# apasarkar/localmd

Hardware: AMD Instinct MI355X
Metric: frames/sec PMD decomposition (higher is better)
Workload: dtype f32; 1 GPU; 512x512x10000_b20; frames=10000, block=20, frames_to_init=10000, max_components=50, parallelism=1 process per GPU

## Files before the change

include/pmd_hip.h:

```cpp
#ifndef PMD_HIP_H
#define PMD_HIP_H
#include <stddef.h>
#include <stdint.h>

#ifdef __cplusplus
extern "C" {
#endif

typedef struct pmd_ctx pmd_ctx;

int pmd_version(void);
int pmd_ctx_create(int device, void* hip_stream, pmd_ctx** out);
int pmd_ctx_destroy(pmd_ctx* ctx);
int pmd_ctx_set_stream(pmd_ctx* ctx, void* hip_stream);
int pmd_ctx_sync(pmd_ctx* ctx);
const char* pmd_last_error(pmd_ctx* ctx);

int pmd_profile_enable(pmd_ctx* ctx, int on);
int pmd_profile_query(pmd_ctx* ctx, const char* name, double* total_ms, int* count);
int pmd_profile_names(pmd_ctx* ctx, char* buf, int cap);

int pmd_tile_dpad(int d);
int pmd_tile_rpad(int r);
long pmd_time_ld(long t);
// ... 101 lines not shown
                      float* R_out, long ldr, float* s_out, float* Vt_out, long ldvt, void* ws, size_t ws_bytes);
int pmd_gram_blocks(pmd_ctx* ctx, const float* Uw, int dpad, int b1, int b2, const int* tile_pix, const int* pairs,
                    int n_pairs, const int* origins, const int* col_off, const int* ranks, int n_tiles, int Rt,
                    const float* basis, long D, int K, float* Gblk, float* Gbg, float* Gstrip, long ldgs);
int pmd_gram_apply(pmd_ctx* ctx, const float* Gblk, const float* Gbg, const float* Gstrip, long ldgs, const int* nbr_ptr,
                   const int* nbr, const int* col_off, const int* ranks, int n_tiles, int Rt, int K, int max_rank,
                   const float* M, long ldm, int ncols, float* GM, long ldgm);
size_t pmd_orthogonalize_factored_workspace_bytes(int m);
int pmd_orthogonalize_factored(pmd_ctx* ctx, const float* M, int Rc, int m, long ldm, const float* GM, long ldgm,
                               float* Et_out, long lde, int* rprime_host, void* ws, size_t ws_bytes);
int pmd_orthogonalize_chol(pmd_ctx* ctx, const float* M, int Rc, int m, long ldm, const float* GM, long ldgm,
                           float* Et_out, long lde, int* ok_host, void* ws, size_t ws_bytes);
size_t pmd_orthogonalize_chol_workspace_bytes(int Rc, int m);
int pmd_psvd_vp_gram(pmd_ctx* ctx, const float* Et, int rp, int m, long lde, const float* W1, int nc, long ldw, int et_lower, float* Vp,
                     long ldv, float* C, long ldc);
size_t pmd_psvd_finish_workspace_bytes(int rp);
int pmd_psvd_finish(pmd_ctx* ctx, float* C, long ldc, int rp, const float* Vp, int nc, long ldv, float* W_out, long ldw, float* s_out,
                    float* Vt_out, long ldvt, void* ws, size_t ws_bytes);
size_t pmd_projected_svd_factored_workspace_bytes(int Rc, int m, int rp, int T);
int pmd_projected_svd_factored(pmd_ctx* ctx, const float* M, int Rc, int m, long ldm, const float* Et, int rp, long lde,
                               const float* Z, int T, long ldz, float* R_out, long ldr, float* s_out, float* Vt_out,
                               long ldvt, float* Vp_out, long ldvp, float* X1_out, const float* W1_in, int et_lower,
                               void* ws, size_t ws_bytes);
size_t pmd_gram_mtgm_workspace_bytes(int rows, int m);
long pmd_gram_mtgm_ld(int rows);
int pmd_gram_mtgm(pmd_ctx* ctx, const float* M, int rows, int m, long ldm, const float* GM, long ldgm, float* C, long ldc,
                  void* ws, size_t ws_bytes);
size_t pmd_chol_inverse_workspace_bytes(int m);
int pmd_chol_inverse(pmd_ctx* ctx, float* C, int m, long ldc, int abs_last_pivot, int* ok_host, void* ws, size_t ws_bytes);
int pmd_transpose(pmd_ctx* ctx, const float* src, long ld_src, int rows, int cols, float* dst, long ld_dst);
// ... 60 lines not shown
```

localmd_amd/_lib.py:

```python
import ctypes as C
import os

_HERE = os.path.dirname(os.path.abspath(__file__))
LIB_PATH = os.environ.get("PMD_HIP_LIB") or os.path.join(_HERE, "libpmd_hip.so")

c_i, c_l, c_f, c_d, c_p = C.c_int, C.c_long, C.c_float, C.c_double, C.c_void_p
c_u64, c_u32, c_sz = C.c_uint64, C.c_uint32, C.c_size_t

SIGNATURES = {
    "pmd_version": (c_i, []),
    "pmd_comm_unique_id": (c_i, [c_p]),
    "pmd_ctx_create": (c_i, [c_i, c_p, C.POINTER(c_p)]),
    "pmd_ctx_destroy": (c_i, [c_p]),
    "pmd_ctx_set_stream": (c_i, [c_p, c_p]),
    "pmd_ctx_sync": (c_i, [c_p]),
    "pmd_last_error": (C.c_char_p, [c_p]),
    "pmd_profile_enable": (c_i, [c_p, c_i]),
    "pmd_profile_query": (c_i, [c_p, C.c_char_p, C.POINTER(c_d), C.POINTER(c_i)]),
    "pmd_profile_names": (c_i, [c_p, C.c_char_p, c_i]),
    "pmd_tile_dpad": (c_i, [c_i]),
    "pmd_tile_rpad": (c_i, [c_i]),
    "pmd_time_ld": (c_l, [c_l]),
    "pmd_rng_normal": (c_i, [c_p, c_u64, c_u32, c_u32, c_u32, c_i, c_l, c_i, c_i, c_p, c_l, c_l]),
    "pmd_stats_workspace_bytes": (c_sz, [c_i, c_l, c_i]),
# ... 56 lines not shown
    "pmd_projected_svd_factored_workspace_bytes": (c_sz, [c_i, c_i, c_i, c_i]),
    "pmd_projected_svd_factored": (c_i, [c_p, c_p, c_i, c_i, c_l, c_p, c_i, c_l, c_p, c_i, c_l, c_p, c_l, c_p, c_p, c_l,
                                         c_p, c_l, c_p, c_p, c_i, c_p, c_sz]),
    "pmd_gram_mtgm_workspace_bytes": (c_sz, [c_i, c_i]),
    "pmd_gram_mtgm_ld": (c_l, [c_i]),
    "pmd_gram_mtgm": (c_i, [c_p, c_p, c_i, c_i, c_l, c_p, c_l, c_p, c_l, c_p, c_sz]),
    "pmd_chol_inverse_workspace_bytes": (c_sz, [c_i]),
    "pmd_chol_inverse": (c_i, [c_p, c_p, c_i, c_l, c_i, C.POINTER(c_i), c_p, c_sz]),
    "pmd_ctx_set_null_cutoff": (c_i, [c_p, C.c_float]),
    "pmd_comm_init": (c_i, [c_p, c_p, c_i, c_i]),
    "pmd_comm_destroy": (c_i, [c_p]),
    "pmd_comm_all_reduce_f32": (c_i, [c_p, c_p, c_sz]),
    "pmd_comm_all_gather": (c_i, [c_p, c_p, c_p, c_sz]),
    "pmd_transpose": (c_i, [c_p, c_p, c_l, c_i, c_i, c_p, c_l]),
    "pmd_psvd_vp_gram": (c_i, [c_p, c_p, c_i, c_i, c_l, c_p, c_i, c_l, c_i, c_p, c_l, c_p, c_l]),
    "pmd_psvd_finish_workspace_bytes": (c_sz, [c_i]),
    "pmd_psvd_finish": (c_i, [c_p, c_p, c_l, c_i, c_p, c_i, c_l, c_p, c_l, c_p, c_p, c_l, c_p, c_sz]),
    "pmd_csr_count": (c_i, [c_p, c_i, c_i, c_i, c_p, c_p, c_i, c_p, c_i, c_p]),
    "pmd_csr_fill": (c_i, [c_p, c_i, c_i, c_i, c_i, c_p, c_p, c_p, c_p, c_i, c_p, c_p, c_p, c_i, c_p, c_p, c_p, c_i, c_i,
                           c_p, c_p, c_p, c_p, c_i]),
    "pmd_scratch_trim": (c_i, [c_p, C.c_size_t]),
    "pmd_gemm_split_active": (c_i, [c_p, c_i, c_i, c_i]),
    "pmd_gemm": (c_i, [c_p, c_i, c_i, c_i, c_i, c_i, c_f, c_p, c_l, c_p, c_l, c_f, c_p, c_l]),
    "pmdk_tile_atx": (c_i, [c_p, c_p, c_l, c_p, c_i, c_l, c_i, c_p, c_l, c_i, c_p, c_l, c_l, c_i, c_i, c_i]),
    "pmdk_tile_atx_rows": (c_i, [c_p, c_p, c_l, c_p, c_i, c_l, c_i, c_p, c_l, c_i, c_p, c_l, c_l, c_i, c_i, c_i, c_i]),
    "pmdk_tile_xbt": (c_i, [c_p, c_p, c_l, c_p, c_i, c_l, c_i, c_p, c_l, c_l, c_p, c_l, c_l, c_i, c_i, c_i, c_i]),
    "pmdk_tile_gram": (c_i, [c_p, c_p, c_l, c_l, c_i, c_i, c_i, c_p]),
    "pmdk_tile_rowmix": (c_i, [c_p, c_p, c_l, c_l, c_p, c_l, c_i, c_i, c_p, c_l, c_l, c_i, c_i]),
    "pmdk_small_qr": (c_i, [c_p, c_p, c_l, c_i, c_i, c_i, c_p, c_l, c_i, c_i]),
    "pmdk_small_eig": (c_i, [c_p, c_p, c_i, c_i, c_i, c_d, c_p, c_p, c_i]),
# ... 138 lines not shown
```

localmd_amd/csrc/capi.hip:

```cpp
#include "pmd_internal.h"
#include "../../include/pmd_hip.h"

#define CTX_CHECK(ctx) \
  if (!(ctx)) return PMD_ERR_ARG;

extern "C" {

int pmd_version(void) { return 1; }

int pmd_ctx_create(int device, void* hip_stream, pmd_ctx** out) {
  if (!out) return PMD_ERR_ARG;
  *out = nullptr;
  int count = 0;
  if (hipGetDeviceCount(&count) != hipSuccess || device < 0 || device >= count) return PMD_ERR_HIP;
  if (hipSetDevice(device) != hipSuccess) return PMD_ERR_HIP;
  pmd_ctx* ctx = new pmd_ctx();
  ctx->device = device;
  ctx->stream = (hipStream_t)hip_stream;
  ctx->tables = nullptr;
  ctx->scratch = nullptr;
  ctx->scratch_bytes = 0;
  ctx->scratch2 = nullptr;
  ctx->scratch2_bytes = 0;
  ctx->atx_ranks = nullptr;
// ... 406 lines not shown
size_t pmd_chol_inverse_workspace_bytes(int m) { return pmd_chol_inverse_workspace_bytes_impl(m); }
int pmd_chol_inverse(pmd_ctx* ctx, float* C, int m, long ldc, int abs_last_pivot, int* ok_host, void* ws, size_t ws_bytes) {
  CTX_CHECK(ctx);
  return pmd_chol_inverse_impl(ctx, C, m, ldc, abs_last_pivot, ok_host, ws, ws_bytes);
}
int pmd_transpose(pmd_ctx* ctx, const float* src, long ld_src, int rows, int cols, float* dst, long ld_dst) {
  CTX_CHECK(ctx);
  return pmd_transpose_impl(ctx, src, ld_src, rows, cols, dst, ld_dst);
}
int pmd_psvd_vp_gram(pmd_ctx* ctx, const float* Et, int rp, int m, long lde, const float* W1, int nc, long ldw, int et_lower, float* Vp,
                     long ldv, float* C, long ldc) {
  CTX_CHECK(ctx);
  if (rp < 1 || m < rp || nc < 0 || ldc < rp) return pmd_fail(ctx, PMD_ERR_ARG, "pmd_psvd_vp_gram", "bad shape");
  return pmd_psvd_vp_gram_impl(ctx, Et, rp, m, lde, W1, nc, ldw, et_lower, Vp, ldv, C, ldc);
}
size_t pmd_psvd_finish_workspace_bytes(int rp) { return pmd_psvd_finish_workspace_bytes_impl(rp); }
int pmd_psvd_finish(pmd_ctx* ctx, float* C, long ldc, int rp, const float* Vp, int nc, long ldv, float* W_out, long ldw, float* s_out,
                    float* Vt_out, long ldvt, void* ws, size_t ws_bytes) {
  CTX_CHECK(ctx);
  if (rp < 1 || nc < 0 || ldc < rp) return pmd_fail(ctx, PMD_ERR_ARG, "pmd_psvd_finish", "bad shape");
  return pmd_psvd_finish_impl(ctx, C, ldc, rp, Vp, nc, ldv, W_out, ldw, s_out, Vt_out, ldvt, ws, ws_bytes);
}
size_t pmd_projected_svd_factored_workspace_bytes(int Rc, int m, int rp, int T) {
  return pmd_projected_svd_factored_workspace_bytes_impl(Rc, m, rp, T);
}
int pmd_projected_svd_factored(pmd_ctx* ctx, const float* M, int Rc, int m, long ldm, const float* Et, int rp, long lde,
                               const float* Z, int T, long ldz, float* R_out, long ldr, float* s_out, float* Vt_out,
                               long ldvt, float* Vp_out, long ldvp, float* X1_out, const float* W1_in, int et_lower,
                               void* ws, size_t ws_bytes) {
  CTX_CHECK(ctx);
// ... 96 lines not shown
```

localmd_amd/csrc/global.hip:

```cpp
#include "pmd_internal.h"
#include <rocsolver/rocsolver.h>
#include <algorithm>
#include <cmath>
#include <vector>

#define RUN(call)                 \
  do {                            \
    int rc__ = (call);            \
    if (rc__ != PMD_OK) return rc__; \
  } while (0)

#define PMD_BLAS(ctx, call)                                                     \
  do {                                                                          \
    rocblas_status s__ = (call);                                                \
    if (s__ != rocblas_status_success) return pmd_fail(ctx, PMD_ERR_BLAS, #call, rocblas_status_to_string(s__)); \
  } while (0)

__global__ void sum_partials_kernel(const float* __restrict__ part, long mn, int n, int S, float beta, float* __restrict__ C, long ldc) {
  for (long i = blockIdx.x * (long)blockDim.x + threadIdx.x; i < mn; i += (long)gridDim.x * blockDim.x) {
    const long r = i / n;
    const int c = (int)(i - r * n);
    float acc = 0.f;
    for (int s = 0; s < S; ++s) acc += part[(long)s * mn + i];
    float* o = C + r * ldc + c;
// ... 356 lines not shown
  PMD_HIP(ctx, hipMemcpyAsync(scale, hscale.data(), (size_t)rp * sizeof(float), hipMemcpyHostToDevice, ctx->stream));
  RUN(launch_gather_rows(ctx, C, ldc, perm, scale, rp, m, Et, m));
  if (M) RUN(pmd_gemm_rm(ctx, 0, 1, R, rp, m, 1.f, M, ldm, Et, m, 0.f, P_out, ldp));
  else RUN(launch_transpose(ctx, Et, m, rp, m, P_out, ldp));
  PMD_HIP(ctx, hipStreamSynchronize(ctx->stream));
  return PMD_OK;
}

size_t pmd_projected_svd_workspace_bytes_impl(int rows_p, int n1, int n2) {
  const size_t nk = (size_t)std::min(n1, n2);
  size_t b = (nk + 4) * nk * sizeof(float) * 2 + nk * (sizeof(float) * 5 + sizeof(int)) + 8192;
  if (n1 > n2) b += (size_t)n1 * n2 * sizeof(float);
  return b + 8192;
}

int pmd_projected_svd_impl(pmd_ctx* ctx, const float* P, int rows_p, long ldp, const float* V, int n1, int n2, long ldv,
                           float* R_out, long ldr, float* s_out, float* Vt_out, long ldvt, void* ws, size_t ws_bytes) {
  const int nk = std::min(n1, n2);
  pmd_arena ar(ws, ws_bytes);
  const long ldc = pmd_round_up(nk, 4);
  float* C = ar.take_n<float>((size_t)ldc * nk);
  float* Wt = ar.take_n<float>((size_t)nk * nk);
  float* w = ar.take_n<float>(nk);
  float* work = ar.take_n<float>(nk);
  float* sgn = ar.take_n<float>(nk);
  float* inv = ar.take_n<float>(nk);
  int* perm = ar.take_n<int>(nk);
  int* info = ar.take_n<int>(4);
  float* left = (n1 > n2) ? ar.take_n<float>((size_t)n1 * n2) : nullptr;
  if (ar.overflow) return pmd_fail(ctx, PMD_ERR_WORKSPACE, "pmd_projected_svd", "workspace too small");
  {
    pmd_prof_scope prof__(ctx, "rocblas_ssyrk");
    const float one = 1.f, zero = 0.f;
    const int kfull = (n1 <= n2) ? n2 : n1;
    const int kc = pmd_gemm_k_chunk(kfull);
    for (int k0 = 0; k0 < kfull; k0 += kc) {
      const int kk = std::min(kc, kfull - k0);
      if (n1 <= n2)
        PMD_BLAS(ctx, rocblas_ssyrk(ctx->blas, rocblas_fill_lower, rocblas_operation_transpose, n1, kk, &one, V + k0, (rocblas_int)ldv,
                                    k0 == 0 ? &zero : &one, C, (rocblas_int)ldc));
      else
        PMD_BLAS(ctx, rocblas_ssyrk(ctx->blas, rocblas_fill_lower, rocblas_operation_none, n2, kk, &one, V + (long)k0 * ldv, (rocblas_int)ldv,
                                    k0 == 0 ? &zero : &one, C, (rocblas_int)ldc));
    }
  }
  RUN(pmd_syevd(ctx, nk, C, ldc, w, work, info));
  std::vector<float> hw(nk);
  int hinfo = 0;
  PMD_HIP(ctx, hipMemcpyAsync(hw.data(), w, (size_t)nk * sizeof(float), hipMemcpyDeviceToHost, ctx->stream));
  PMD_HIP(ctx, hipMemcpyAsync(&hinfo, info, sizeof(int), hipMemcpyDeviceToHost, ctx->stream));
  PMD_HIP(ctx, hipStreamSynchronize(ctx->stream));
  if (hinfo != 0) return pmd_fail(ctx, PMD_ERR_BLAS, "rocsolver_ssyevd", "did not converge");
  std::vector<int> idx(nk);
  for (int i = 0; i < nk; ++i) idx[i] = i;
  std::stable_sort(idx.begin(), idx.end(), [&](int a, int b) { return std::fabs(hw[a]) > std::fabs(hw[b]); });
  std::vector<float> hs(nk), hsgn(nk), hinv(nk);
  for (int i = 0; i < nk; ++i) {
    const float lam = hw[idx[i]];
// ... 11 lines not shown
    hipLaunchKernelGGL(scale_rows2_kernel, dim3(8, nk), dim3(256), 0, ctx->stream, Vt_out, ldvt, n2, inv);
    PMD_LAUNCH_CHECK(ctx, "scale_rows2_kernel");
    if (P) RUN(pmd_gemm_rm(ctx, 0, 1, rows_p, nk, n1, 1.f, P, ldp, Wt, nk, 0.f, R_out, ldr));
    else RUN(launch_transpose(ctx, Wt, nk, nk, n1, R_out, ldr));
  } else {
    RUN(pmd_gemm_rm(ctx, 0, 1, n1, nk, n2, 1.f, V, ldv, Wt, nk, 0.f, left, nk));
    hipLaunchKernelGGL(scale_cols_kernel, dim3(8, n1), dim3(256), 0, ctx->stream, left, (long)nk, nk, inv);
    PMD_LAUNCH_CHECK(ctx, "scale_cols_kernel");
    RUN(pmd_gemm_rm(ctx, 0, 0, rows_p, nk, n1, 1.f, P, ldp, left, nk, 0.f, R_out, ldr));
    PMD_HIP(ctx, hipMemcpy2DAsync(Vt_out, ldvt * sizeof(float), Wt, (size_t)nk * sizeof(float), (size_t)nk * sizeof(float), nk, hipMemcpyDeviceToDevice, ctx->stream));
  }
  PMD_HIP(ctx, hipStreamSynchronize(ctx->stream));
  return PMD_OK;
}

static int psvd_gram_rows(pmd_ctx* ctx, const float* V, int n1, int n2, long ldv, float* C, long ldc) {
  pmd_prof_scope prof__(ctx, "rocblas_ssyrk");
  const float one = 1.f, zero = 0.f;
  const int kc = pmd_gemm_k_chunk(n2);
  if (n2 <= 0) { PMD_HIP(ctx, hipMemsetAsync(C, 0, (size_t)n1 * ldc * sizeof(float), ctx->stream)); return PMD_OK; }
  for (int k0 = 0; k0 < n2; k0 += kc) {
    const int kk = std::min(kc, n2 - k0);
    PMD_BLAS(ctx, rocblas_ssyrk(ctx->blas, rocblas_fill_lower, rocblas_operation_transpose, n1, kk, &one, V + k0, (rocblas_int)ldv,
                                k0 == 0 ? &zero : &one, C, (rocblas_int)ldc));
  }
  return PMD_OK;
}

int pmd_psvd_vp_gram_impl(pmd_ctx* ctx, const float* Et, int rp, int m, long lde, const float* W1, int nc, long ldw, int et_lower,
                          float* Vp, long ldv, float* C, long ldc) {
  if (nc > 0) {
    const bool tri = et_lower && rp == m && !pmd_f16x2_wanted(ctx, rp, nc, m);
    const float one = 1.f;
    if (tri) {
      pmd_prof_scope prof__(ctx, "rocblas_strmm");
      PMD_BLAS(ctx, rocblas_strmm(ctx->blas, rocblas_side_right, rocblas_fill_upper, rocblas_operation_none, rocblas_diagonal_non_unit, nc, m,
                                  &one, Et, (rocblas_int)lde, W1, (rocblas_int)ldw, Vp, (rocblas_int)ldv));
    } else {
      RUN(pmd_gemm_rm(ctx, 0, 0, rp, nc, m, 1.f, Et, lde, W1, ldw, 0.f, Vp, ldv));
    }
  }
  return psvd_gram_rows(ctx, Vp, rp, nc, ldv, C, ldc);
}

size_t pmd_psvd_finish_workspace_bytes_impl(int rp) {
  return (size_t)rp * rp * sizeof(float) + (size_t)rp * (sizeof(float) * 5 + sizeof(int)) + 16384;
}

int pmd_psvd_finish_impl(pmd_ctx* ctx, float* C, long ldc, int rp, const float* Vp, int nc, long ldv, float* W_out, long ldw, float* s_out,
                         float* Vt_out, long ldvt, void* ws, size_t ws_bytes) {
  pmd_arena ar(ws, ws_bytes);
  float* Wt = ar.take_n<float>((size_t)rp * rp);
  float* w = ar.take_n<float>(rp);
  float* work = ar.take_n<float>(rp);
  float* sgn = ar.take_n<float>(rp);
  float* inv = ar.take_n<float>(rp);
  int* perm = ar.take_n<int>(rp);
// ... 503 lines not shown
  pmd_arena ar(ws, ws_bytes);
  float* W1 = ar.take_n<float>((size_t)m * T);
  float* Vp = Vp_out ? Vp_out : ar.take_n<float>((size_t)rp * T);
  const long ldv = Vp_out ? ldvp : T;
  float* X1 = X1_out ? X1_out : ar.take_n<float>((size_t)m * rp);
  const long ldt = pmd_round_up(Rc, 64);
  float* Mt = ar.take_n<float>((size_t)m * ldt);
  const size_t sub_bytes = pmd_projected_svd_workspace_bytes_impl(1, rp, T);
  void* sub = ar.take(sub_bytes);
  if (ar.overflow) return pmd_fail(ctx, PMD_ERR_WORKSPACE, "pmd_projected_svd_factored", "workspace too small");
  if (!W1_in) {
    RUN(launch_transpose(ctx, M, ldm, Rc, m, Mt, ldt));
    RUN(pmd_gemm_rm(ctx, 0, 0, m, T, Rc, 1.f, Mt, ldt, Z, ldz, 0.f, W1, T));
  }
  const bool tri_any = et_lower && rp == m;
  const bool tri = tri_any && !pmd_f16x2_wanted(ctx, rp, T, m);
  const float one = 1.f;
  if (tri) {
    pmd_prof_scope prof__(ctx, "rocblas_strmm");
    PMD_BLAS(ctx, rocblas_strmm(ctx->blas, rocblas_side_right, rocblas_fill_upper, rocblas_operation_none,
                                rocblas_diagonal_non_unit, T, m, &one, Et, (rocblas_int)lde, W1_in ? W1_in : W1, T, Vp,
                                (rocblas_int)ldv));
  } else {
    RUN(pmd_gemm_rm(ctx, 0, 0, rp, T, m, 1.f, Et, lde, W1_in ? W1_in : W1, T, 0.f, Vp, ldv));
  }
  float* Wmat = W1;
  RUN(pmd_projected_svd_impl(ctx, nullptr, 0, 0, Vp, rp, T, ldv, Wmat, rp, s_out, Vt_out, ldvt, sub, sub_bytes));
  if (tri_any && !pmd_f16x2_wanted(ctx, m, rp, rp)) {
    pmd_prof_scope prof__(ctx, "rocblas_strmm");
    PMD_BLAS(ctx, rocblas_strmm(ctx->blas, rocblas_side_right, rocblas_fill_upper, rocblas_operation_transpose,
                                rocblas_diagonal_non_unit, rp, m, &one, Et, (rocblas_int)lde, Wmat, rp, X1, rp));
  } else {
    RUN(pmd_gemm_rm(ctx, 1, 0, m, rp, rp, 1.f, Et, lde, Wmat, rp, 0.f, X1, rp));
  }
  if (R_out) RUN(pmd_gemm_rm(ctx, 0, 0, Rc, rp, m, 1.f, M, ldm, X1, rp, 0.f, R_out, ldr));
  return PMD_OK;
}

#define CHOL_NB 128
#define CHOL_LS (CHOL_NB + 1)
__global__ __launch_bounds__(256) void potf2_block_kernel(float* __restrict__ A, long ld, int nb, int k0, int* __restrict__ info,
                                                          int n_abs_last, float* __restrict__ linv_out) {
  extern __shared__ float chol_dyn[];
  __shared__ float s_col[2][CHOL_NB];
  const int tid = threadIdx.x;
  const int tr = tid >> 4, tc = tid & 15;
  float a[8][8];
#pragma unroll
  for (int i = 0; i < 8; ++i)
// ... 431 lines not shown
```

localmd_amd/csrc/pmd_internal.h:

```cpp
#pragma once
#include "pmd_common.h"

int pmd_init_tables(pmd_ctx* ctx);
extern "C" {
int pmd_tile_dpad(int d);
long pmd_time_ld(long t);
size_t pmd_stats_workspace_bytes(int T, long D, int frame_const);
size_t pmd_stats_stream_workspace_bytes(int T, long D);
}

int pmd_launch_rng(pmd_ctx* ctx, uint64_t seed, uint32_t stream, uint32_t index0, uint32_t index_step, int batch,
                   long rows, int cols, int transpose, float* out, long ld, long batch_stride);

int pmd_launch_stats(pmd_ctx* ctx, const float* movie, int T, long D, int frame_const, int do_noise, float* mean_out,
                     float* std_out, void* ws, size_t ws_bytes);
int pmd_launch_standardize_transpose(pmd_ctx* ctx, const float* movie, long D, const int* frames, int nf,
                                     const float* mean, const float* stdv, float* out, long ld);
int pmd_launch_stats_stream_accumulate(pmd_ctx* ctx, const void* batch, int elem, int t0, int nb, int T, long D,
                                       int do_noise, void* ws, size_t ws_bytes);
int pmd_launch_stats_stream_finish(pmd_ctx* ctx, int T, long D, int do_noise, float* mean_out, float* std_out, void* ws,
                                   size_t ws_bytes);
int pmd_launch_standardize_transpose_typed(pmd_ctx* ctx, const void* movie, int elem, long D, const int* frames, int nf,
                                           const float* mean, const float* stdv, float* out, long ld);
int pmd_launch_gather_frames(pmd_ctx* ctx, const void* src, int elem, long D, const int* src_rows, const int* dst_rows,
// ... 152 lines not shown
int pmd_csr_fill_impl(pmd_ctx* ctx, int d1, int d2, int order_f, int b1, const int* cover1, const int* cover2,
                      const int* orig1, const int* orig2, int n2, const int* ranks, const int* col_off, const float* Ut,
                      int dpad, const float* w, const double* inv_cumw, const float* basis, int K, int Rt,
                      const long* indptr, double* data, int* indices, int* zero_count, int rpad);
size_t pmd_orthogonalize_factored_workspace_bytes_impl(int m);
int pmd_orthogonalize_factored_impl(pmd_ctx* ctx, const float* M, int Rc, int m, long ldm, const float* GM, long ldgm,
                                    float* Et_out, long lde, int* rprime_out, void* ws, size_t ws_bytes);
size_t pmd_projected_svd_factored_workspace_bytes_impl(int Rc, int m, int rp, int T);
size_t pmd_orthogonalize_chol_workspace_bytes_impl(int Rc, int m);
int pmd_projected_svd_factored_impl(pmd_ctx* ctx, const float* M, int Rc, int m, long ldm, const float* Et, int rp,
                                    long lde, const float* Z, int T, long ldz, float* R_out, long ldr, float* s_out,
                                    float* Vt_out, long ldvt, float* Vp_out, long ldvp, float* X1_out,
                                    const float* W1_in, int et_lower, void* ws, size_t ws_bytes);
int pmd_psvd_vp_gram_impl(pmd_ctx* ctx, const float* Et, int rp, int m, long lde, const float* W1, int nc, long ldw, int et_lower,
                          float* Vp, long ldv, float* C, long ldc);
size_t pmd_psvd_finish_workspace_bytes_impl(int rp);
int pmd_psvd_finish_impl(pmd_ctx* ctx, float* C, long ldc, int rp, const float* Vp, int nc, long ldv, float* W_out, long ldw, float* s_out,
                         float* Vt_out, long ldvt, void* ws, size_t ws_bytes);
long pmd_gram_mtgm_ld_impl(int rows);
size_t pmd_gram_mtgm_workspace_bytes_impl(int rows, int m);
int pmd_gram_mtgm_impl(pmd_ctx* ctx, const float* M, int rows, int m, long ldm, const float* GM, long ldgm, float* C,
                       long ldc, void* ws, size_t ws_bytes);
size_t pmd_chol_inverse_workspace_bytes_impl(int m);
int pmd_chol_inverse_impl(pmd_ctx* ctx, float* C, int m, long ldc, int abs_last_pivot, int* ok_host, void* ws, size_t ws_bytes);
int pmd_transpose_impl(pmd_ctx* ctx, const float* src, long lds_, int rows, int cols, float* dst, long ldd);
int pmd_orthogonalize_chol_impl(pmd_ctx* ctx, const float* M, int Rc, int m, long ldm, const float* GM, long ldgm,
                                float* Et_out, long lde, int* ok_host, void* ws, size_t ws_bytes);

int pmd_launch_bin_average(pmd_ctx* ctx, const float* X, long ldx, long n_rows, int a, int nbins, float* xbar, long ldb);
int pmd_launch_tile_cross_gram(pmd_ctx* ctx, const float* A, const float* B, long tile_stride, int ld, int len,
// ... 15 lines not shown
```

localmd_amd/csrc/sytrd.hip:

```cpp
#include "pmd_internal.h"
#include <rocsolver/rocsolver.h>
#include <algorithm>
#include <cmath>
#include <cstdlib>
#include <vector>

#define PMD_BLAS(ctx, call)                                                     \
  do {                                                                          \
    rocblas_status s__ = (call);                                                \
    if (s__ != rocblas_status_success) return pmd_fail(ctx, PMD_ERR_BLAS, #call, rocblas_status_to_string(s__)); \
  } while (0)

namespace {

constexpr int NB = 64;
constexpr int BR = 64;
constexpr int CW = 1024;
constexpr int DCH = 256;

struct sytrd_bufs {
  float* W;
  long ldw;
  float* RP;
  float* CP;
// ... 586 lines not shown
    if (ok) *reinterpret_cast<float4*>(B.CP + (long)b * B.ldp + pos) = make_float4(col[0], col[1], col[2], col[3]);
  }
  for (int o = 32; o > 0; o >>= 1) spart += __shfl_xor(spart, o);
  if (lane == 0) s_red[wave] = spart;
  __syncthreads();
  if (tid == 0) {
    float tot = 0.f;
    for (int t = 0; t < 8; ++t) tot += s_red[t];
    B.SP[wg] = tot;
  }
  TRACE_STAMP(5);
}

typedef float f32x4 __attribute__((ext_vector_type(4)));

__global__ __launch_bounds__(256) void sytrd_rank2k_lds_kernel(float* __restrict__ A, long lda, int n, int ts, int j0, int nbc,
                                                               const float* __restrict__ W, long ldw) {
  constexpr int LS = 68;
  __shared__ float sv_c[32][LS], sw_c[32][LS], sv_r[32][LS], sw_r[32][LS];
  const int I = blockIdx.y, J = blockIdx.x;
  if (J < I) return;
  const int tid = threadIdx.x, lane = tid & 63, wave = __builtin_amdgcn_readfirstlane((int)(tid >> 6));
  const int n16 = lane & 15, kk = lane >> 4;
  const int cb = ts + 64 * I, r0 = ts + 64 * J;
  const int c0 = cb + 16 * wave;
  const float* V = A + (long)j0 * lda;
  f32x4 acc[4];
#pragma unroll
  for (int jn = 0; jn < 4; ++jn) acc[jn] = (f32x4){0.f, 0.f, 0.f, 0.f};
  const int lp = tid & 63, lk = tid >> 6;
  const int pc = min(cb + lp, n - 1), pr = min(r0 + lp, n - 1);
  for (int h = 0; h < 2; ++h) {
    if (h) __syncthreads();
#pragma unroll
    for (int u = 0; u < 8; ++u) {
      const int k = 32 * h + lk + 4 * u;
      const bool in = k < nbc;
      const long kc = in ? k : 0;
      const float v1 = V[kc * lda + pc], w1 = W[kc * ldw + pc], v2 = V[kc * lda + pr], w2 = W[kc * ldw + pr];
      sv_c[lk + 4 * u][lp] = in ? v1 : 0.f;
      sw_c[lk + 4 * u][lp] = in ? w1 : 0.f;
      sv_r[lk + 4 * u][lp] = in ? v2 : 0.f;
      sw_r[lk + 4 * u][lp] = in ? w2 : 0.f;
    }
    __syncthreads();
    if (c0 < n) {
#pragma unroll
      for (int k0 = 0; k0 < 32; k0 += 4) {
        const int k = k0 + kk;
        const float a1 = sv_c[k][16 * wave + n16], a2 = sw_c[k][16 * wave + n16];
#pragma unroll
        for (int jn = 0; jn < 4; ++jn) {
          const float b1 = sw_r[k][16 * jn + n16], b2 = sv_r[k][16 * jn + n16];
          acc[jn] = __builtin_amdgcn_mfma_f32_16x16x4f32(a1, b1, acc[jn], 0, 0, 0);
          acc[jn] = __builtin_amdgcn_mfma_f32_16x16x4f32(a2, b2, acc[jn], 0, 0, 0);
        }
      }
    }
  }
  if (c0 >= n) return;
#pragma unroll
  for (int jn = 0; jn < 4; ++jn) {
    const int col = r0 + 16 * jn + n16;
#pragma unroll
    for (int i = 0; i < 4; ++i) {
      const int row = c0 + 4 * kk + i;
      if (row < n && col < n && col >= row) A[(long)row * lda + col] -= acc[jn][i];
    }
  }
}

__global__ __launch_bounds__(256) void sytrd_rank2k_kernel(float* __restrict__ A, long lda, int n, int ts, int j0, int nbc,
                                                           const float* __restrict__ W, long ldw) {
  const int I = blockIdx.y, J = blockIdx.x;
  if (J < I) return;
  const int lane = threadIdx.x & 63, wave = __builtin_amdgcn_readfirstlane((int)(threadIdx.x >> 6));
  const int n16 = lane & 15, kk = lane >> 4;
  const int c0 = ts + 64 * I + 16 * wave, r0 = ts + 64 * J;
  if (c0 >= n) return;
  const float* V = A + (long)j0 * lda;
  const int c = min(c0 + n16, n - 1);
  int r[4];
// ... 59 lines not shown
    S[(long)i * kb + jj] = v;
  }
}

}

constexpr int QB = 1024;

size_t pmd_apply_q_workspace_bytes_impl(int n) {
  return ((size_t)QB * n + (size_t)QB * QB + (size_t)n * QB) * sizeof(float) + 4096;
}

int pmd_apply_q_impl(pmd_ctx* ctx, int n, const float* A, long lda, const float* tau, float* Z, long ldz, void* ws,
                     size_t ws_bytes) {
  return pmd_apply_q_off_impl(ctx, n, A, lda, tau, Z, ldz, ws, ws_bytes, 1);
}

int pmd_apply_q_off_impl(pmd_ctx* ctx, int n, const float* A, long lda, const float* tau, float* Z, long ldz, void* ws,
                         size_t ws_bytes, int off) {
  pmd_prof_scope prof__(ctx, "apply_q");
  if (n < off + 1) return PMD_OK;
  pmd_arena ar(ws, ws_bytes);
  float* Vb = ar.take_n<float>((size_t)QB * n);
  float* S = ar.take_n<float>((size_t)QB * QB);
  float* Y = ar.take_n<float>((size_t)n * QB);
  if (ar.overflow) return pmd_fail(ctx, PMD_ERR_WORKSPACE, "pmd_apply_q", "workspace too small");
  const int nref = n - off;
  const float one = 1.f;
  for (int k0 = (nref - 1) / QB * QB; k0 >= 0; k0 -= QB) {
    const int kb = std::min(QB, nref - k0);
    const int p0 = k0 + off, np = n - p0;
    hipLaunchKernelGGL(extract_v_kernel, dim3((np + 255) / 256, kb), dim3(256), 0, ctx->stream, A, lda, tau, k0, p0, np, Vb, (long)np, off);
    PMD_LAUNCH_CHECK(ctx, "extract_v_kernel");
    int rc = pmd_gemm_rm(ctx, 0, 1, kb, kb, np, 1.f, Vb, np, Vb, np, 0.f, S, kb);
    if (rc != PMD_OK) return rc;
    hipLaunchKernelGGL(tinv_kernel, dim3(kb), dim3(256), 0, ctx->stream, S, kb, tau, k0);
    PMD_LAUNCH_CHECK(ctx, "tinv_kernel");
    rc = pmd_gemm_rm(ctx, 0, 1, n, kb, np, 1.f, Z + p0, ldz, Vb, np, 0.f, Y, kb);
    if (rc != PMD_OK) return rc;
    PMD_BLAS(ctx, rocblas_strsm(ctx->blas, rocblas_side_left, rocblas_fill_lower, rocblas_operation_transpose,
                                rocblas_diagonal_non_unit, kb, n, &one, S, kb, Y, kb));
    rc = pmd_gemm_rm(ctx, 0, 0, n, np, kb, -1.f, Y, kb, Vb, np, 1.f, Z + p0, ldz);
    if (rc != PMD_OK) return rc;
  }
  return PMD_OK;
}

size_t pmd_sytrd_workspace_bytes_impl(int n) {
  const size_t n4 = (size_t)pmd_round_up(n, 4);
  const size_t nq = (size_t)(n / 256 + 2), nbk = (size_t)(n / BR + 2);
  size_t b = 0;
  b += NB * n4 * sizeof(float) + 256;
  b += nq * n4 * sizeof(float) + 256;
  b += nbk * n4 * sizeof(float) + 256;
  b += (nq + 2) * (nbk + 2) * sizeof(float) + 256;
  b += (size_t)(n / DCH + 2) * 2 * NB * sizeof(float) + 256;
  b += (size_t)(n / 32 + 2) * sizeof(double) + 256;
// ... 69 lines not shown
    PMD_LAUNCH_CHECK(ctx, "sytrd panel");
    const int ts = j0 + nbc;
    if (adv_old)
      hipLaunchKernelGGL((sytrd_advance_kernel<true, false>), dim3((n - ts + APOS - 1) / APOS), dim3(320), 0, st, A, lda, n, ts, j0, B, nsp, d);
    else
      hipLaunchKernelGGL((sytrd_advance2_kernel<false>), dim3((n - ts + APOS2 - 1) / APOS2), dim3(448), 0, st, A, lda, n, ts, j0, B, nsp, d);
    PMD_LAUNCH_CHECK(ctx, "sytrd_advance_kernel");
    if (use_rocblas_syr2k) {
      PMD_BLAS(ctx, rocblas_ssyr2k(ctx->blas, rocblas_fill_lower, rocblas_operation_none, n - ts, nbc, &minus1,
                                   A + (long)j0 * lda + ts, (rocblas_int)lda, B.W + ts, (rocblas_int)B.ldw, &one,
                                   A + (long)ts * lda + ts, (rocblas_int)lda));
    } else {
      const int nt = (n - ts + 63) / 64;
      static int r2k_lds = -1;
      if (r2k_lds < 0) { const char* e = getenv("PMD_RANK2K"); r2k_lds = (e && !strcmp(e, "direct")) ? 0 : 1; }
      if (r2k_lds) hipLaunchKernelGGL(sytrd_rank2k_lds_kernel, dim3(nt, nt), dim3(256), 0, st, A, lda, n, ts, j0, nbc, B.W, B.ldw);
      else hipLaunchKernelGGL(sytrd_rank2k_kernel, dim3(nt, nt), dim3(256), 0, st, A, lda, n, ts, j0, nbc, B.W, B.ldw);
      PMD_LAUNCH_CHECK(ctx, "sytrd_rank2k_kernel");
    }
  }
  hipLaunchKernelGGL((sytrd_advance_kernel<false, false>), dim3(1), dim3(320), 0, st, A, lda, n, n - 1, n - 1, B, 0, d);
  PMD_LAUNCH_CHECK(ctx, "sytrd_advance_kernel");
  return PMD_OK;
}

int pmd_sytrd_rocsolver(pmd_ctx* ctx, int n, float* A, long lda, float* d, float* e, float* tau) {
  pmd_prof_scope prof__(ctx, "rocsolver_ssytrd");
  PMD_BLAS(ctx, rocsolver_ssytrd(ctx->blas, rocblas_fill_lower, n, A, (rocblas_int)lda, d, e, tau));
  return PMD_OK;
}

// ... 254 lines not shown
```

Baseline: 16420 frames/s.

## Route triangular and Gram products through blocked f16x2 split GEMMs; compact rank2k grid

```diff
diff --git a/include/pmd_hip.h b/include/pmd_hip.h
--- a/include/pmd_hip.h
+++ b/include/pmd_hip.h
@@ -139,6 +139,9 @@
 size_t pmd_orthogonalize_chol_workspace_bytes(int Rc, int m);
 int pmd_psvd_vp_gram(pmd_ctx* ctx, const float* Et, int rp, int m, long lde, const float* W1, int nc, long ldw, int et_lower, float* Vp,
                      long ldv, float* C, long ldc);
+int pmd_gram_rows(pmd_ctx* ctx, const float* V, int n1, int n2, long ldv, float* C, long ldc);
+int pmd_tri_lower_matmul(pmd_ctx* ctx, int trans, const float* Et, int n, long lde, const float* W, int nc, long ldw, float* Out,
+                         long ldo);
 size_t pmd_psvd_finish_workspace_bytes(int rp);
 int pmd_psvd_finish(pmd_ctx* ctx, float* C, long ldc, int rp, const float* Vp, int nc, long ldv, float* W_out, long ldw, float* s_out,
                     float* Vt_out, long ldvt, void* ws, size_t ws_bytes);
diff --git a/localmd_amd/_lib.py b/localmd_amd/_lib.py
--- a/localmd_amd/_lib.py
+++ b/localmd_amd/_lib.py
@@ -94,6 +94,8 @@
     "pmd_comm_all_gather": (c_i, [c_p, c_p, c_p, c_sz]),
     "pmd_transpose": (c_i, [c_p, c_p, c_l, c_i, c_i, c_p, c_l]),
     "pmd_psvd_vp_gram": (c_i, [c_p, c_p, c_i, c_i, c_l, c_p, c_i, c_l, c_i, c_p, c_l, c_p, c_l]),
+    "pmd_gram_rows": (c_i, [c_p, c_p, c_i, c_i, c_l, c_p, c_l]),
+    "pmd_tri_lower_matmul": (c_i, [c_p, c_i, c_p, c_i, c_l, c_p, c_i, c_l, c_p, c_l]),
     "pmd_psvd_finish_workspace_bytes": (c_sz, [c_i]),
     "pmd_psvd_finish": (c_i, [c_p, c_p, c_l, c_i, c_p, c_i, c_l, c_p, c_l, c_p, c_p, c_l, c_p, c_sz]),
     "pmd_csr_count": (c_i, [c_p, c_i, c_i, c_i, c_p, c_p, c_i, c_p, c_i, c_p]),
diff --git a/localmd_amd/csrc/capi.hip b/localmd_amd/csrc/capi.hip
--- a/localmd_amd/csrc/capi.hip
+++ b/localmd_amd/csrc/capi.hip
@@ -444,6 +444,18 @@
   if (rp < 1 || m < rp || nc < 0 || ldc < rp) return pmd_fail(ctx, PMD_ERR_ARG, "pmd_psvd_vp_gram", "bad shape");
   return pmd_psvd_vp_gram_impl(ctx, Et, rp, m, lde, W1, nc, ldw, et_lower, Vp, ldv, C, ldc);
 }
+int pmd_gram_rows(pmd_ctx* ctx, const float* V, int n1, int n2, long ldv, float* C, long ldc) {
+  CTX_CHECK(ctx);
+  if (!V || !C || n1 < 1 || n2 < 0 || ldv < n2 || ldc < n1) return pmd_fail(ctx, PMD_ERR_ARG, "pmd_gram_rows", "bad argument");
+  return pmd_gram_rows_impl(ctx, V, n1, n2, ldv, C, ldc);
+}
+int pmd_tri_lower_matmul(pmd_ctx* ctx, int trans, const float* Et, int n, long lde, const float* W, int nc, long ldw, float* Out,
+                         long ldo) {
+  CTX_CHECK(ctx);
+  if (!Et || !W || !Out || Out == W || n < 1 || nc < 1 || lde < n || ldw < nc || ldo < nc)
+    return pmd_fail(ctx, PMD_ERR_ARG, "pmd_tri_lower_matmul", "bad argument");
+  return pmd_tri_lower_matmul_impl(ctx, trans, Et, n, lde, W, nc, ldw, Out, ldo);
+}
 size_t pmd_psvd_finish_workspace_bytes(int rp) { return pmd_psvd_finish_workspace_bytes_impl(rp); }
 int pmd_psvd_finish(pmd_ctx* ctx, float* C, long ldc, int rp, const float* Vp, int nc, long ldv, float* W_out, long ldw, float* s_out,
                     float* Vt_out, long ldvt, void* ws, size_t ws_bytes) {
diff --git a/localmd_amd/csrc/global.hip b/localmd_amd/csrc/global.hip
--- a/localmd_amd/csrc/global.hip
+++ b/localmd_amd/csrc/global.hip
@@ -394,6 +394,111 @@
   return b + 8192;
 }
 
+static int tri_block_rows(int n) {
+  static int nblk = -1;
+  if (nblk < 0) { const char* e = getenv("PMD_TRI_BLOCKS"); nblk = e ? std::max(1, atoi(e)) : 5; }
+  return std::max(256, ((n + nblk - 1) / nblk + 255) / 256 * 256);
+}
+
+static pmd_f16x2_op piece_view(const pmd_f16x2_op& o, long row, long col) {
+  pmd_f16x2_op v = o;
+  const long off = row * o.ld + col;
+  v.h1 += off;
+  v.h2 += off;
+  if (v.h3) v.h3 += off;
+  return v;
+}
+
+int pmd_gram_rows_f16x2(pmd_ctx* ctx, const float* V, int n1, int n2, long ldv, float* C, long ldc, int* done) {
+  *done = 0;
+  const int bs = tri_block_rows(n1);
+  if (n1 <= 0 || n2 <= 0 || !pmd_f16x2_wanted(ctx, std::min(bs, n1), n1, n2) || pmd_is_host_pointer(C)) return PMD_OK;
+  void* w = nullptr;
+  RUN(pmd_split_scratch(ctx, pmd_f16x2_bytes(n1, n2, 2), &w));
+  if (!w) return PMD_OK;
+  pmd_f16x2_op v;
+  int usable = 0;
+  RUN(pmd_f16x2_split(ctx, 1, &V, &n1, &n2, &ldv, &w, &v, &usable, 2));
+  if (!usable) return PMD_OK;
+  static int kch_env = -2;
+  if (kch_env == -2) { const char* e = getenv("PMD_F16X2_GRAM_KCHUNK"); kch_env = e ? atoi(e) : -1; }
+  const int kch = kch_env > 0 ? kch_env : (kch_env == 0 ? n2 : pmd_gemm_k_chunk(n2));
+  for (int i0 = 0; i0 < n1; i0 += bs) {
+    const int nr = std::min(bs, n1 - i0);
+    for (int k0 = 0; k0 < n2; k0 += kch) {
+      const int kk = std::min(kch, n2 - k0);
+      const pmd_f16x2_op a = piece_view(v, i0, k0);
+      int ok = 0;
+      RUN(pmd_f16x2_matmul(ctx, 0, 1, nr, n1 - i0, kk, 1.f, a, a, k0 ? 1.f : 0.f, C + (long)i0 * ldc + i0, ldc, &ok));
+      if (!ok) return PMD_OK;
+    }
+  }
+  *done = 1;
+  return PMD_OK;
+}
+
+int pmd_tri_lower_f16x2(pmd_ctx* ctx, int trans, const float* Et, int n, long lde, const float* W, int nc, long ldw, float* Out,
+                        long ldo, int* done) {
+  *done = 0;
+  if (n <= 0 || nc <= 0 || pmd_is_host_pointer(Out)) return PMD_OK;
+  const size_t na = pmd_f16x2_bytes(n, n, 2), nb = pmd_f16x2_bytes(n, nc, 2);
+  void* w = nullptr;
+  RUN(pmd_split_scratch(ctx, na + nb, &w));
+  if (!w) return PMD_OK;
+  const float* X[2] = {Et, W};
+  const int rows[2] = {n, n}, cols[2] = {n, nc};
+  const long ld[2] = {lde, ldw};
+  void* buf[2] = {w, (char*)w + na};
+  pmd_f16x2_op ops[2];
+  int usable = 0;
+  RUN(pmd_f16x2_split(ctx, 2, X, rows, cols, ld, buf, ops, &usable, 2));
+  if (!usable) return PMD_OK;
+  const int bs = tri_block_rows(n);
+  for (int i0 = 0; i0 < n; i0 += bs) {
+    const int nr = std::min(bs, n - i0);
+    int ok = 0;
+    if (!trans)
+      RUN(pmd_f16x2_matmul(ctx, 0, 0, nr, nc, i0 + nr, 1.f, piece_view(ops[0], i0, 0), ops[1], 0.f, Out + (long)i0 * ldo, ldo, &ok));
+    else
+      RUN(pmd_f16x2_matmul(ctx, 1, 0, nr, nc, n - i0, 1.f, piece_view(ops[0], i0, i0), piece_view(ops[1], i0, 0), 0.f,
+                           Out + (long)i0 * ldo, ldo, &ok));
+    if (!ok) return PMD_OK;
+  }
+  *done = 1;
+  return PMD_OK;
+}
+
+int pmd_tri_lower_matmul_impl(pmd_ctx* ctx, int trans, const float* Et, int n, long lde, const float* W, int nc, long ldw, float* Out,
+                              long ldo) {
+  if (pmd_f16x2_wanted(ctx, n, nc, n)) {
+    int done = 0;
+    RUN(pmd_tri_lower_f16x2(ctx, trans, Et, n, lde, W, nc, ldw, Out, ldo, &done));
+    if (done) return PMD_OK;
+    return pmd_gemm_rm(ctx, trans, 0, n, nc, n, 1.f, Et, lde, W, ldw, 0.f, Out, ldo);
+  }
+  pmd_prof_scope prof__(ctx, "rocblas_strmm");
+  const float one = 1.f;
+  PMD_BLAS(ctx, rocblas_strmm(ctx->blas, rocblas_side_right, rocblas_fill_upper, trans ? rocblas_operation_transpose : rocblas_operation_none,
+                              rocblas_diagonal_non_unit, nc, n, &one, Et, (rocblas_int)lde, W, (rocblas_int)ldw, Out, (rocblas_int)ldo));
+  return PMD_OK;
+}
+
+int pmd_gram_rows_impl(pmd_ctx* ctx, const float* V, int n1, int n2, long ldv, float* C, long ldc) {
+  if (n2 <= 0) { PMD_HIP(ctx, hipMemsetAsync(C, 0, (size_t)n1 * ldc * sizeof(float), ctx->stream)); return PMD_OK; }
+  int done = 0;
+  RUN(pmd_gram_rows_f16x2(ctx, V, n1, n2, ldv, C, ldc, &done));
+  if (done) return PMD_OK;
+  pmd_prof_scope prof__(ctx, "rocblas_ssyrk");
+  const float one = 1.f, zero = 0.f;
+  const int kc = pmd_gemm_k_chunk(n2);
+  for (int k0 = 0; k0 < n2; k0 += kc) {
+    const int kk = std::min(kc, n2 - k0);
+    PMD_BLAS(ctx, rocblas_ssyrk(ctx->blas, rocblas_fill_lower, rocblas_operation_transpose, n1, kk, &one, V + k0, (rocblas_int)ldv,
+                                k0 == 0 ? &zero : &one, C, (rocblas_int)ldc));
+  }
+  return PMD_OK;
+}
+
 int pmd_projected_svd_impl(pmd_ctx* ctx, const float* P, int rows_p, long ldp, const float* V, int n1, int n2, long ldv,
                            float* R_out, long ldr, float* s_out, float* Vt_out, long ldvt, void* ws, size_t ws_bytes) {
   const int nk = std::min(n1, n2);
@@ -409,19 +514,16 @@
   int* info = ar.take_n<int>(4);
   float* left = (n1 > n2) ? ar.take_n<float>((size_t)n1 * n2) : nullptr;
   if (ar.overflow) return pmd_fail(ctx, PMD_ERR_WORKSPACE, "pmd_projected_svd", "workspace too small");
-  {
+  if (n1 <= n2) {
+    RUN(pmd_gram_rows_impl(ctx, V, n1, n2, ldv, C, ldc));
+  } else {
     pmd_prof_scope prof__(ctx, "rocblas_ssyrk");
     const float one = 1.f, zero = 0.f;
-    const int kfull = (n1 <= n2) ? n2 : n1;
-    const int kc = pmd_gemm_k_chunk(kfull);
-    for (int k0 = 0; k0 < kfull; k0 += kc) {
-      const int kk = std::min(kc, kfull - k0);
-      if (n1 <= n2)
-        PMD_BLAS(ctx, rocblas_ssyrk(ctx->blas, rocblas_fill_lower, rocblas_operation_transpose, n1, kk, &one, V + k0, (rocblas_int)ldv,
-                                    k0 == 0 ? &zero : &one, C, (rocblas_int)ldc));
-      else
-        PMD_BLAS(ctx, rocblas_ssyrk(ctx->blas, rocblas_fill_lower, rocblas_operation_none, n2, kk, &one, V + (long)k0 * ldv, (rocblas_int)ldv,
-                                    k0 == 0 ? &zero : &one, C, (rocblas_int)ldc));
+    const int kc = pmd_gemm_k_chunk(n1);
+    for (int k0 = 0; k0 < n1; k0 += kc) {
+      const int kk = std::min(kc, n1 - k0);
+      PMD_BLAS(ctx, rocblas_ssyrk(ctx->blas, rocblas_fill_lower, rocblas_operation_none, n2, kk, &one, V + (long)k0 * ldv, (rocblas_int)ldv,
+                                  k0 == 0 ? &zero : &one, C, (rocblas_int)ldc));
     }
   }
   RUN(pmd_syevd(ctx, nk, C, ldc, w, work, info));
@@ -463,33 +565,13 @@
   return PMD_OK;
 }
 
-static int psvd_gram_rows(pmd_ctx* ctx, const float* V, int n1, int n2, long ldv, float* C, long ldc) {
-  pmd_prof_scope prof__(ctx, "rocblas_ssyrk");
-  const float one = 1.f, zero = 0.f;
-  const int kc = pmd_gemm_k_chunk(n2);
-  if (n2 <= 0) { PMD_HIP(ctx, hipMemsetAsync(C, 0, (size_t)n1 * ldc * sizeof(float), ctx->stream)); return PMD_OK; }
-  for (int k0 = 0; k0 < n2; k0 += kc) {
-    const int kk = std::min(kc, n2 - k0);
-    PMD_BLAS(ctx, rocblas_ssyrk(ctx->blas, rocblas_fill_lower, rocblas_operation_transpose, n1, kk, &one, V + k0, (rocblas_int)ldv,
-                                k0 == 0 ? &zero : &one, C, (rocblas_int)ldc));
-  }
-  return PMD_OK;
-}
-
 int pmd_psvd_vp_gram_impl(pmd_ctx* ctx, const float* Et, int rp, int m, long lde, const float* W1, int nc, long ldw, int et_lower,
                           float* Vp, long ldv, float* C, long ldc) {
   if (nc > 0) {
-    const bool tri = et_lower && rp == m && !pmd_f16x2_wanted(ctx, rp, nc, m);
-    const float one = 1.f;
-    if (tri) {
-      pmd_prof_scope prof__(ctx, "rocblas_strmm");
-      PMD_BLAS(ctx, rocblas_strmm(ctx->blas, rocblas_side_right, rocblas_fill_upper, rocblas_operation_none, rocblas_diagonal_non_unit, nc, m,
-                                  &one, Et, (rocblas_int)lde, W1, (rocblas_int)ldw, Vp, (rocblas_int)ldv));
-    } else {
-      RUN(pmd_gemm_rm(ctx, 0, 0, rp, nc, m, 1.f, Et, lde, W1, ldw, 0.f, Vp, ldv));
-    }
-  }
-  return psvd_gram_rows(ctx, Vp, rp, nc, ldv, C, ldc);
+    if (et_lower && rp == m) RUN(pmd_tri_lower_matmul_impl(ctx, 0, Et, m, lde, W1, nc, ldw, Vp, ldv));
+    else RUN(pmd_gemm_rm(ctx, 0, 0, rp, nc, m, 1.f, Et, lde, W1, ldw, 0.f, Vp, ldv));
+  }
+  return pmd_gram_rows_impl(ctx, Vp, rp, nc, ldv, C, ldc);
 }
 
 size_t pmd_psvd_finish_workspace_bytes_impl(int rp) {
@@ -1023,25 +1105,12 @@
     RUN(pmd_gemm_rm(ctx, 0, 0, m, T, Rc, 1.f, Mt, ldt, Z, ldz, 0.f, W1, T));
   }
   const bool tri_any = et_lower && rp == m;
-  const bool tri = tri_any && !pmd_f16x2_wanted(ctx, rp, T, m);
-  const float one = 1.f;
-  if (tri) {
-    pmd_prof_scope prof__(ctx, "rocblas_strmm");
-    PMD_BLAS(ctx, rocblas_strmm(ctx->blas, rocblas_side_right, rocblas_fill_upper, rocblas_operation_none,
-                                rocblas_diagonal_non_unit, T, m, &one, Et, (rocblas_int)lde, W1_in ? W1_in : W1, T, Vp,
-                                (rocblas_int)ldv));
-  } else {
-    RUN(pmd_gemm_rm(ctx, 0, 0, rp, T, m, 1.f, Et, lde, W1_in ? W1_in : W1, T, 0.f, Vp, ldv));
-  }
+  if (tri_any) RUN(pmd_tri_lower_matmul_impl(ctx, 0, Et, m, lde, W1_in ? W1_in : W1, T, T, Vp, ldv));
+  else RUN(pmd_gemm_rm(ctx, 0, 0, rp, T, m, 1.f, Et, lde, W1_in ? W1_in : W1, T, 0.f, Vp, ldv));
   float* Wmat = W1;
   RUN(pmd_projected_svd_impl(ctx, nullptr, 0, 0, Vp, rp, T, ldv, Wmat, rp, s_out, Vt_out, ldvt, sub, sub_bytes));
-  if (tri_any && !pmd_f16x2_wanted(ctx, m, rp, rp)) {
-    pmd_prof_scope prof__(ctx, "rocblas_strmm");
-    PMD_BLAS(ctx, rocblas_strmm(ctx->blas, rocblas_side_right, rocblas_fill_upper, rocblas_operation_transpose,
-                                rocblas_diagonal_non_unit, rp, m, &one, Et, (rocblas_int)lde, Wmat, rp, X1, rp));
-  } else {
-    RUN(pmd_gemm_rm(ctx, 1, 0, m, rp, rp, 1.f, Et, lde, Wmat, rp, 0.f, X1, rp));
-  }
+  if (tri_any) RUN(pmd_tri_lower_matmul_impl(ctx, 1, Et, m, lde, Wmat, rp, rp, X1, rp));
+  else RUN(pmd_gemm_rm(ctx, 1, 0, m, rp, rp, 1.f, Et, lde, Wmat, rp, 0.f, X1, rp));
   if (R_out) RUN(pmd_gemm_rm(ctx, 0, 0, Rc, rp, m, 1.f, M, ldm, X1, rp, 0.f, R_out, ldr));
   return PMD_OK;
 }
diff --git a/localmd_amd/csrc/pmd_internal.h b/localmd_amd/csrc/pmd_internal.h
--- a/localmd_amd/csrc/pmd_internal.h
+++ b/localmd_amd/csrc/pmd_internal.h
@@ -190,6 +190,12 @@
                                     const float* W1_in, int et_lower, void* ws, size_t ws_bytes);
 int pmd_psvd_vp_gram_impl(pmd_ctx* ctx, const float* Et, int rp, int m, long lde, const float* W1, int nc, long ldw, int et_lower,
                           float* Vp, long ldv, float* C, long ldc);
+int pmd_gram_rows_f16x2(pmd_ctx* ctx, const float* V, int n1, int n2, long ldv, float* C, long ldc, int* done);
+int pmd_gram_rows_impl(pmd_ctx* ctx, const float* V, int n1, int n2, long ldv, float* C, long ldc);
+int pmd_tri_lower_f16x2(pmd_ctx* ctx, int trans, const float* Et, int n, long lde, const float* W, int nc, long ldw, float* Out,
+                        long ldo, int* done);
+int pmd_tri_lower_matmul_impl(pmd_ctx* ctx, int trans, const float* Et, int n, long lde, const float* W, int nc, long ldw, float* Out,
+                              long ldo);
 size_t pmd_psvd_finish_workspace_bytes_impl(int rp);
 int pmd_psvd_finish_impl(pmd_ctx* ctx, float* C, long ldc, int rp, const float* Vp, int nc, long ldv, float* W_out, long ldw, float* s_out,
                          float* Vt_out, long ldvt, void* ws, size_t ws_bytes);
diff --git a/localmd_amd/csrc/sytrd.hip b/localmd_amd/csrc/sytrd.hip
--- a/localmd_amd/csrc/sytrd.hip
+++ b/localmd_amd/csrc/sytrd.hip
@@ -624,34 +624,58 @@
 
 typedef float f32x4 __attribute__((ext_vector_type(4)));
 
-__global__ __launch_bounds__(256) void sytrd_rank2k_lds_kernel(float* __restrict__ A, long lda, int n, int ts, int j0, int nbc,
+__global__ __launch_bounds__(256) __attribute__((amdgpu_waves_per_eu(4, 4))) void sytrd_rank2k_lds_kernel(float* __restrict__ A, long lda, int n, int ts, int j0, int nbc,
                                                                const float* __restrict__ W, long ldw) {
   constexpr int LS = 68;
   __shared__ float sv_c[32][LS], sw_c[32][LS], sv_r[32][LS], sw_r[32][LS];
-  const int I = blockIdx.y, J = blockIdx.x;
-  if (J < I) return;
+  const int t = blockIdx.x;
+  int J = (int)((sqrtf(8.f * (float)t + 1.f) - 1.f) * 0.5f);
+  while (J * (J + 1) / 2 > t) --J;
+  while ((J + 1) * (J + 2) / 2 <= t) ++J;
+  const int I = t - J * (J + 1) / 2;
   const int tid = threadIdx.x, lane = tid & 63, wave = __builtin_amdgcn_readfirstlane((int)(tid >> 6));
   const int n16 = lane & 15, kk = lane >> 4;
   const int cb = ts + 64 * I, r0 = ts + 64 * J;
   const int c0 = cb + 16 * wave;
   const float* V = A + (long)j0 * lda;
-  f32x4 acc[4];
-#pragma unroll
-  for (int jn = 0; jn < 4; ++jn) acc[jn] = (f32x4){0.f, 0.f, 0.f, 0.f};
+  float at[4][4];
+#pragma unroll
+  for (int jn = 0; jn < 4; ++jn) {
+    const int col = r0 + 16 * jn + n16;
+#pragma unroll
+    for (int i = 0; i < 4; ++i) {
+      const int row = c0 + 4 * kk + i;
+      at[jn][i] = (row < n && col < n && col >= row) ? A[(long)row * lda + col] : 0.f;
+    }
+  }
   const int lp = tid & 63, lk = tid >> 6;
   const int pc = min(cb + lp, n - 1), pr = min(r0 + lp, n - 1);
-  for (int h = 0; h < 2; ++h) {
-    if (h) __syncthreads();
+  float pv1[2][8], pw1[2][8], pv2[2][8], pw2[2][8];
+#pragma unroll
+  for (int h = 0; h < 2; ++h)
 #pragma unroll
     for (int u = 0; u < 8; ++u) {
       const int k = 32 * h + lk + 4 * u;
       const bool in = k < nbc;
       const long kc = in ? k : 0;
       const float v1 = V[kc * lda + pc], w1 = W[kc * ldw + pc], v2 = V[kc * lda + pr], w2 = W[kc * ldw + pr];
-      sv_c[lk + 4 * u][lp] = in ? v1 : 0.f;
-      sw_c[lk + 4 * u][lp] = in ? w1 : 0.f;
-      sv_r[lk + 4 * u][lp] = in ? v2 : 0.f;
-      sw_r[lk + 4 * u][lp] = in ? w2 : 0.f;
+      pv1[h][u] = in ? v1 : 0.f;
+      pw1[h][u] = in ? w1 : 0.f;
+      pv2[h][u] = in ? v2 : 0.f;
+      pw2[h][u] = in ? w2 : 0.f;
+    }
+  f32x4 acc[4];
+#pragma unroll
+  for (int jn = 0; jn < 4; ++jn) acc[jn] = (f32x4){0.f, 0.f, 0.f, 0.f};
+#pragma unroll
+  for (int h = 0; h < 2; ++h) {
+    if (h) __syncthreads();
+#pragma unroll
+    for (int u = 0; u < 8; ++u) {
+      sv_c[lk + 4 * u][lp] = pv1[h][u];
+      sw_c[lk + 4 * u][lp] = pw1[h][u];
+      sv_r[lk + 4 * u][lp] = pv2[h][u];
+      sw_r[lk + 4 * u][lp] = pw2[h][u];
     }
     __syncthreads();
     if (c0 < n) {
@@ -675,7 +699,7 @@
 #pragma unroll
     for (int i = 0; i < 4; ++i) {
       const int row = c0 + 4 * kk + i;
-      if (row < n && col < n && col >= row) A[(long)row * lda + col] -= acc[jn][i];
+      if (row < n && col < n && col >= row) A[(long)row * lda + col] = at[jn][i] - acc[jn][i];
     }
   }
 }
@@ -765,6 +789,18 @@
 int pmd_apply_q_impl(pmd_ctx* ctx, int n, const float* A, long lda, const float* tau, float* Z, long ldz, void* ws,
                      size_t ws_bytes) {
   return pmd_apply_q_off_impl(ctx, n, A, lda, tau, Z, ldz, ws, ws_bytes, 1);
+}
+
+static int apply_q_gemm(pmd_ctx* ctx, int transB, int m, int n, int k, float alpha, const float* A, long lda, const float* B, long ldb,
+                        float beta, float* C, long ldc) {
+  if (ctx->gemm_split && !pmd_f16x2_wanted(ctx, m, n, k) && std::min(m, std::min(n, k)) >= ctx->gemm_split_min_dim &&
+      2.0 * m * (double)n * k >= 0.3 * ctx->gemm_split_min_flop && !pmd_is_host_pointer(C)) {
+    int done = 0;
+    const int rc = pmd_gemm_f16x2(ctx, 0, transB, m, n, k, alpha, A, lda, B, ldb, beta, C, ldc, &done);
+    if (rc != PMD_OK) return rc;
+    if (done) return PMD_OK;
+  }
+  return pmd_gemm_rm(ctx, 0, transB, m, n, k, alpha, A, lda, B, ldb, beta, C, ldc);
 }
 
 int pmd_apply_q_off_impl(pmd_ctx* ctx, int n, const float* A, long lda, const float* tau, float* Z, long ldz, void* ws,
@@ -787,11 +823,11 @@
     if (rc != PMD_OK) return rc;
     hipLaunchKernelGGL(tinv_kernel, dim3(kb), dim3(256), 0, ctx->stream, S, kb, tau, k0);
     PMD_LAUNCH_CHECK(ctx, "tinv_kernel");
-    rc = pmd_gemm_rm(ctx, 0, 1, n, kb, np, 1.f, Z + p0, ldz, Vb, np, 0.f, Y, kb);
+    rc = apply_q_gemm(ctx, 1, n, kb, np, 1.f, Z + p0, ldz, Vb, np, 0.f, Y, kb);
     if (rc != PMD_OK) return rc;
     PMD_BLAS(ctx, rocblas_strsm(ctx->blas, rocblas_side_left, rocblas_fill_lower, rocblas_operation_transpose,
                                 rocblas_diagonal_non_unit, kb, n, &one, S, kb, Y, kb));
-    rc = pmd_gemm_rm(ctx, 0, 0, n, np, kb, -1.f, Y, kb, Vb, np, 1.f, Z + p0, ldz);
+    rc = apply_q_gemm(ctx, 0, n, np, kb, -1.f, Y, kb, Vb, np, 1.f, Z + p0, ldz);
     if (rc != PMD_OK) return rc;
   }
   return PMD_OK;
@@ -891,7 +927,7 @@
       const int nt = (n - ts + 63) / 64;
       static int r2k_lds = -1;
       if (r2k_lds < 0) { const char* e = getenv("PMD_RANK2K"); r2k_lds = (e && !strcmp(e, "direct")) ? 0 : 1; }
-      if (r2k_lds) hipLaunchKernelGGL(sytrd_rank2k_lds_kernel, dim3(nt, nt), dim3(256), 0, st, A, lda, n, ts, j0, nbc, B.W, B.ldw);
+      if (r2k_lds) hipLaunchKernelGGL(sytrd_rank2k_lds_kernel, dim3(nt * (nt + 1) / 2), dim3(256), 0, st, A, lda, n, ts, j0, nbc, B.W, B.ldw);
       else hipLaunchKernelGGL(sytrd_rank2k_kernel, dim3(nt, nt), dim3(256), 0, st, A, lda, n, ts, j0, nbc, B.W, B.ldw);
       PMD_LAUNCH_CHECK(ctx, "sytrd_rank2k_kernel");
     }
```

Result: faster. 16660 frames/s, median of 6 (+1.5%).
